# saidwivedi/InteractVLM

Measured on AMD Instinct MI355X. Metric: images/sec end-to-end contact inference, higher is better.
Workload: dtype f16

## Files before the change

### include/ivlm_hip.h

```cpp
#ifndef IVLM_HIP_H
#define IVLM_HIP_H

#include <stddef.h>
#include <stdint.h>

#ifdef __cplusplus
extern "C" {
#endif

#define IVLM_OK 0
#define IVLM_ERR_INVALID_ARG (-1)
#define IVLM_ERR_WORKSPACE (-2)
#define IVLM_ERR_LAUNCH (-3)
#define IVLM_ERR_UNSUPPORTED (-4)

#define IVLM_F32 0
#define IVLM_BF16 1
#define IVLM_BF16_SPLIT 2
#define IVLM_F16 4
#define IVLM_F16_SPLIT 5
#define IVLM_FP8 3

#define IVLM_GEMM_A_F32 1
#define IVLM_GEMM_RES_F32 2
// ... 314 lines not shown
int ivlm_pack_bf12m_fill(const void *w, int N_valid, int n_rows, int K, const int32_t *ebase, const int32_t *patch_ptr, void *Pf, void *Ef,
                         int32_t *patch_col, void *patch_val, ivlm_stream_t stream);
int ivlm_gemv16_bf12m(const float *x, int64_t lda, int M, const void *Pf, const void *Ef, const int32_t *ebase,
                      const int32_t *patch_ptr, const int32_t *patch_col, const void *patch_val, void *C, int64_t ldc, const void *bias,
                      const void *residual, int64_t ldr, int N, int K, int act, int out_f32, const void *rms_w, float rms_eps, int flags,
                      ivlm_stream_t stream);
void ivlm_gemv16_bf12m_tuning(int tiles_per_block);
int ivlm_decode_parts_tuning(int ranges);
void ivlm_gemv1_bf12m_tuning(int wide_max_blocks);
int ivlm_gemv1_bf12m_staging(int form);
int ivlm_unpack_bf12(const void *P, int64_t ldp, const void *E, int64_t lde, const int32_t *ebase, const int32_t *patch_ptr,
                     const int32_t *patch_col, const void *patch_val, int N, int K, void *w_out, ivlm_stream_t stream);

int ivlm_argmax_f32(const float *x, int rows, int cols, int32_t *out, ivlm_stream_t stream);
int ivlm_argmax_f32_bump(const float *x, int rows, int cols, int32_t *out, int32_t *bump, ivlm_stream_t stream);

int ivlm_im2col_nchw(const void *x, void *out, int B, int C, int H, int W, int ks, int stride, int Kpad,
                     ivlm_stream_t stream);
int ivlm_im2col3x3_nhwc(const void *x, void *out, int B, int H, int W, int C, ivlm_stream_t stream);
int ivlm_im2col3x3_nhwc_strided(const void *x, int64_t ldx, void *out, int64_t ldo, int B, int H, int W, int C,
                                ivlm_stream_t stream);
int ivlm_gather_rows(void *dst, int dst_kind, int64_t ldd, const void *src, int src_dtype, int64_t lds, const int32_t *idx,
                     const void *add, int add_dtype, int64_t lda, int64_t rows, int cols, const float *fp8_scale,
                     ivlm_stream_t stream);
int ivlm_amax(const void *x, int dtype, int64_t n, float *out, ivlm_stream_t stream);
int ivlm_add_rows(void *out, int out_kind, const void *a, int a_dtype, const void *b, int b_dtype, int64_t rows, int cols,
                  int64_t b_rows, int op, ivlm_stream_t stream);
int ivlm_fill_rows(void *dst, int64_t ldd, const int32_t *idx, int64_t n_idx, const void *row, int cols,
                   ivlm_stream_t stream);
int ivlm_dense_pe(const void *gauss, void *pe, int pe_dtype, int h, int w, int F, ivlm_stream_t stream);
// ... 181 lines not shown
```

### interactvlm_amd/csrc/elementwise.hip

```cpp
#include "kernels.h"

namespace ivlm {
namespace {

constexpr int kT = 256;

inline int grid_for(int64_t work_items, int max_blocks = 8192) {
    int64_t b = (work_items + kT - 1) / kT;
    if (b < 1) b = 1;
    return (int)(b < max_blocks ? b : max_blocks);
}

__global__ __launch_bounds__(kT) void im2col_nchw_kernel(const bf16_t* __restrict__ x, bf16_t* __restrict__ out, int B,
                                                         int C, int H, int W, int ks, int stride, int Kpad) {
    const int gh = (H - ks) / stride + 1, gw = (W - ks) / stride + 1;
    const int K = C * ks * ks;
    const int64_t total = (int64_t)B * gh * gw * (Kpad >> 3);
    for (int64_t i = (int64_t)blockIdx.x * kT + threadIdx.x; i < total; i += (int64_t)gridDim.x * kT) {
        const int c8 = (int)(i % (Kpad >> 3));
        const int64_t row = i / (Kpad >> 3);
        const int gx = (int)(row % gw), gy = (int)((row / gw) % gh), b = (int)(row / ((int64_t)gw * gh));
        bf16_t v[8];
#pragma unroll
        for (int e = 0; e < 8; ++e) {
// ... 84 lines not shown
    const float inv_scale = scale ? 1.0f / *scale : 1.0f;
    for (int64_t i = (int64_t)blockIdx.x * kT + threadIdx.x; i < total; i += (int64_t)gridDim.x * kT) {
        const int c8 = (int)(i % c8n);
        const int64_t r = i / c8n;
        const int64_t s = idx ? (int64_t)idx[r] : r;
        float v[8] = {0.f, 0.f, 0.f, 0.f, 0.f, 0.f, 0.f, 0.f};
        if (s >= 0) load8(src, src_kind, s * lds_ + c8 * 8, v);
        if (add) {
            float a[8];
            load8(add, add_kind, r * lda + c8 * 8, a);
#pragma unroll
            for (int j = 0; j < 8; ++j) v[j] += a[j];
        }
        store8(dst, dst_kind, r * ldd + c8 * 8, cols, v, inv_scale);
    }
}

__global__ __launch_bounds__(kT) void amax_kernel(const void* __restrict__ x, int kind, int64_t n8, float* __restrict__ out) {
    float m = 0.0f;
    for (int64_t i = (int64_t)blockIdx.x * kT + threadIdx.x; i < n8; i += (int64_t)gridDim.x * kT) {
        float v[8];
        load8(x, kind, i * 8, v);
#pragma unroll
        for (int j = 0; j < 8; ++j) m = fmaxf(m, fabsf(v[j]));
    }
    m = wave_max(m);
    if ((threadIdx.x & 63) == 0) atomicMax(reinterpret_cast<unsigned int*>(out), __float_as_uint(m));
}

__global__ __launch_bounds__(kT) void fill_rows_kernel(bf16_t* __restrict__ dst, int64_t ldd, const int32_t* __restrict__ idx,
// ... 313 lines not shown
    ivlm_enter();
    return ivlm::im2col3x3_nhwc(CBF(x), BF(out), B, H, W, C, ivlm_stream(s));
}
int ivlm_im2col3x3_nhwc_strided(const void* x, int64_t ldx, void* out, int64_t ldo, int B, int H, int W, int C, ivlm_stream_t s) {
    ivlm_enter();
    return ivlm::im2col3x3_nhwc(CBF(x), BF(out), B, H, W, C, ivlm_stream(s), ldx, ldo);
}
int ivlm_gather_rows(void* dst, int dst_kind, int64_t ldd, const void* src, int src_dtype, int64_t lds_, const int32_t* idx,
                     const void* add, int add_dtype, int64_t lda, int64_t rows, int cols, const float* fp8_scale,
                     ivlm_stream_t s) {
    ivlm_enter();
    const int k = dst_kind == IVLM_F32 ? 1 : (dst_kind == IVLM_BF16 ? 0 : (dst_kind == IVLM_BF16_SPLIT ? 2 : (dst_kind == IVLM_FP8 ? 3 : -1)));
    return ivlm::gather_rows(dst, k, ldd, src, src_dtype == IVLM_F32, lds_, idx, add, add_dtype == IVLM_F32, lda, rows, cols,
                             ivlm_stream(s), fp8_scale);
}
int ivlm_amax(const void* x, int dtype, int64_t n, float* out, ivlm_stream_t s) {
    ivlm_enter();
    return ivlm::amax(x, dtype == IVLM_F32, n, out, ivlm_stream(s));
}
int ivlm_add_rows(void* out, int out_kind, const void* a, int a_dtype, const void* b, int b_dtype, int64_t rows, int cols,
                  int64_t b_rows, int op, ivlm_stream_t s) {
    ivlm_enter();
    return ivlm::add_rows(out, out_kind == IVLM_F32 ? 1 : (out_kind == IVLM_BF16 ? 0 : (out_kind == IVLM_BF16_SPLIT ? 2 : -1)),
                          a, a_dtype == IVLM_F32, b, b_dtype == IVLM_F32, rows, cols, b_rows, ivlm_stream(s), op);
}
int ivlm_fill_rows(void* dst, int64_t ldd, const int32_t* idx, int64_t n_idx, const void* row, int cols, ivlm_stream_t s) {
    ivlm_enter();
    return ivlm::fill_rows(BF(dst), ldd, idx, n_idx, CBF(row), cols, ivlm_stream(s));
}
int ivlm_dense_pe(const void* gauss, void* pe, int pe_dtype, int h, int w, int F, ivlm_stream_t s) {
// ... 44 lines not shown
```

### interactvlm_amd/csrc/gemv.hip

```cpp
#include <stdlib.h>

#include <algorithm>

#include "gemv_common.h"

namespace ivlm {
namespace {

constexpr int kMaxM = 8;

__device__ __forceinline__ float dot8(const u32x4_t& w, const u32x4_t& x) {
    float acc = 0.0f;
#pragma unroll
    for (int j = 0; j < 4; ++j) {
        acc += __uint_as_float(w[j] << 16) * __uint_as_float(x[j] << 16);
        acc += __uint_as_float(w[j] & 0xffff0000u) * __uint_as_float(x[j] & 0xffff0000u);
    }
    return acc;
}

__device__ __forceinline__ float dot8f(const u32x4_t& w, const f32x4v_t& xa, const f32x4v_t& xb) {
    float acc = __uint_as_float(w[0] << 16) * xa[0];
    acc = fmaf(__uint_as_float(w[0] & 0xffff0000u), xa[1], acc);
    acc = fmaf(__uint_as_float(w[1] << 16), xa[2], acc);
// ... 295 lines not shown

static int launch_gemv1(const GemmArgs& g, hipStream_t st) {
    int ks = g_gemv1_ksplit > 0 ? g_gemv1_ksplit : 1;
    if (g.act == ACT_SWIGLU || g.K < 2048) ks = 1;
    if (ks == 2) {
        if (g.rms_w) launch_gemv1_ks<true, 2>(g, st);
        else launch_gemv1_ks<false, 2>(g, st);
    } else {
        if (g.rms_w) launch_gemv1_ks<true, 1>(g, st);
        else launch_gemv1_ks<false, 1>(g, st);
    }
    return ivlm_launch_status();
}

__global__ __launch_bounds__(1024) void argmax_kernel(const float* __restrict__ x, int cols, int32_t* __restrict__ out,
                                                      int32_t* __restrict__ bump) {
    __shared__ float sv[16];
    __shared__ int si[16];
    const float* r = x + (int64_t)blockIdx.x * cols;
    float best = -INFINITY;
    int bi = 0x7fffffff;
    auto take = [&](float v, int i) {
        if (v > best || (v == best && i < bi)) {
            best = v;
            bi = i;
        }
    };
    const int head = (int)(((16 - ((uintptr_t)r & 15)) & 15) >> 2);
    const int nhead = head < cols ? head : cols;
    if ((int)threadIdx.x < nhead) take(r[threadIdx.x], threadIdx.x);
    const int nvec = (cols - nhead) >> 2;
    const float4* rv = reinterpret_cast<const float4*>(r + nhead);
    for (int i = threadIdx.x; i < nvec; i += 1024) {
// ... 15 lines not shown
        }
    }
    if ((threadIdx.x & 63) == 0) {
        sv[threadIdx.x >> 6] = best;
        si[threadIdx.x >> 6] = bi;
    }
    __syncthreads();
    if (threadIdx.x == 0) {
        for (int w = 1; w < 16; ++w)
            if (sv[w] > best || (sv[w] == best && si[w] < bi)) {
                best = sv[w];
                bi = si[w];
            }
        out[blockIdx.x] = bi;
        if (bump) bump[blockIdx.x] += 1;
    }
}

}

int g_gemv_max_blocks_per_cu = 0, g_gemv_rows2_min_n = 0;
int g_gemv_legacy = 0;
static int gemv_cu_count() {
    static int cus = 0;
    if (cus == 0) {
        int dev = 0;
        if (hipGetDevice(&dev) != hipSuccess || hipDeviceGetAttribute(&cus, hipDeviceAttributeMultiprocessorCount, dev) != hipSuccess ||
            cus <= 0)
            cus = 256;
    }
// ... 51 lines not shown
        case 7: return launch_gemv<7>(g, st);
        default: return launch_gemv<8>(g, st);
    }
}

int gemv1_fp8w(const GemmArgs& g, hipStream_t st) {
    if (!g.A || !g.W || !g.C || !g.scale_w || g.M != 1 || !g.a_f32 || g.N <= 0 || g.K <= 0) return IVLM_ERR_INVALID_ARG;
    if ((g.K & 15) || (g.ldw & 15) || (size_t)g.K * 4 > 60 * 1024) return IVLM_ERR_UNSUPPORTED;
    if (g.act == ACT_SWIGLU && ((g.N & 1) || g.residual)) return IVLM_ERR_UNSUPPORTED;
    const dim3 grid((g.N + kG1Waves - 1) / kG1Waves), block(64 * kG1Waves);
    if (g.rms_w) ivlm_launch_lds_cap<gemv1_fp8w_kernel<true>>(64 * 1024, grid, block, (size_t)g.K * 4, st, g);
    else ivlm_launch_lds_cap<gemv1_fp8w_kernel<false>>(64 * 1024, grid, block, (size_t)g.K * 4, st, g);
    return ivlm_launch_status();
}

int argmax_f32(const float* x, int rows, int cols, int32_t* out, hipStream_t st, int32_t* bump) {
    if (!x || !out || rows <= 0 || cols <= 0) return IVLM_ERR_INVALID_ARG;
    argmax_kernel<<<rows, 1024, 0, st>>>(x, cols, out, bump);
    return ivlm_launch_status();
}

}

extern "C" int ivlm_gemv_tuning(int max_blocks_per_cu, int rows2_min_n) {
    ivlm::g_gemv_legacy = max_blocks_per_cu < 0 ? 1 : 0;
    ivlm::g_gemv_max_blocks_per_cu = max_blocks_per_cu > 0 ? max_blocks_per_cu : 0;
    ivlm::g_gemv_rows2_min_n = rows2_min_n;
    return 0;
}

extern "C" void ivlm_gemv1_tuning(int ksplit) { ivlm::g_gemv1_ksplit = ksplit; }
extern "C" void ivlm_gemv1_lds_floor(int bytes) { ivlm::g_gemv1_lds_floor = bytes < 0 ? 0 : (bytes > 128 * 1024 ? 128 * 1024 : bytes); }

// ... 5 lines not shown
    g.W = static_cast<const bf16_t*>(Wq);
    g.ldw = ldw;
    g.scale_w = scale_w;
    return ivlm::gemv1_fp8w(g, ivlm_stream(stream));
}

extern "C" int ivlm_argmax_f32(const float* x, int rows, int cols, int32_t* out, ivlm_stream_t stream) {
    ivlm_enter();
    return ivlm::argmax_f32(x, rows, cols, out, ivlm_stream(stream), nullptr);
}

extern "C" int ivlm_argmax_f32_bump(const float* x, int rows, int cols, int32_t* out, int32_t* bump, ivlm_stream_t stream) {
    ivlm_enter();
    return ivlm::argmax_f32(x, rows, cols, out, ivlm_stream(stream), bump);
}
```

### interactvlm_amd/csrc/kernels.h

```cpp
#pragma once
#include "ivlm_common.h"

namespace ivlm {

enum Act : int { ACT_NONE = 0, ACT_GELU = 1, ACT_QUICK_GELU = 2, ACT_RELU = 3, ACT_SILU = 4, ACT_SWIGLU = 5, ACT_SIGMOID = 6 };

struct SplitKFused {
    int32_t* count = nullptr;
    void* C = nullptr;
    const bf16_t* bias = nullptr;
    const bf16_t* residual = nullptr;
    int64_t ldc = 0, ldr = 0, c_lo = 0;
    int res_mod = 0, act = 0, out_f32 = 0, out_f16 = 0, out_split = 0, res_f32 = 0;
};
constexpr int kSplitKCounters = 4096;

struct GemmArgs {
    const bf16_t* A = nullptr;
    const bf16_t* W = nullptr;
    void* C = nullptr;
    const bf16_t* bias = nullptr;
    const bf16_t* residual = nullptr;
    int64_t lda = 0, ldw = 0, ldc = 0, ldr = 0;
    int res_mod = 0;
// ... 20 lines not shown
    float rms_eps = 0.0f;
    SplitKFused sk;
};

GemmArgs gemm_args(const void* A, int64_t lda, const void* W, int64_t ldw, void* C, int64_t ldc, const void* bias, const void* residual,
                   int64_t ldr, int res_mod, int M, int N, int K, int act, int out_f32, int flags, const int32_t* out_rows = nullptr,
                   const int32_t* a_rows = nullptr);
int gemm_bf16(const GemmArgs& g, hipStream_t st);
int gemm_splitk_choice(int M, int N, int K, int act, int has_rms);
int gemm_bf16_splitk(const GemmArgs& g, int splits, float* workspace, size_t ws_bytes, hipStream_t st, int32_t* counters = nullptr);
int linear_bf16(const GemmArgs& g, hipStream_t st);

int layernorm(const void* x, int x_f32, const bf16_t* w, const bf16_t* b, void* y, int y_f32, int64_t rows, int cols, float eps,
              hipStream_t st, int gelu = 0, const int32_t* out_rows = nullptr, const float* fp8_scale = nullptr);
int rmsnorm(const void* x, int x_f32, const bf16_t* w, void* y, int y_f32, int64_t rows, int cols, float eps, hipStream_t st,
            const float* fp8_scale = nullptr);

struct AttnArgs {
    const bf16_t *q, *k, *v;
    bf16_t* o;
    int64_t q_bs, q_hs, q_rs;
    int64_t k_bs, k_hs, k_rs;
    int64_t v_bs, v_hs, v_rs;
    int64_t o_bs, o_hs, o_rs;
    int B, H, Sq, Sk, D;
    float scale;
    int causal;
    int q_pos0;
    const float* rel_h;
    const float* rel_w;
    int rel_kh, rel_kw;
// ... 143 lines not shown
int decode_attn(DecodeAttnForm form, const DecodeAttnArgs& a, hipStream_t st);
bool attn_oproj_fits(int H, int D, int cus);
size_t llama_decode_attn_splitkv_scratch_bytes(int H, int D);
size_t llama_decode_attn_batch_prefix_scratch_bytes(int B, int H, int D);

extern int g_decode_parts_S;
constexpr int kDecodePartsMaxS = 4;
__host__ __device__ constexpr int decode_parts_stride(int D) { return D + 4; }

int spec_accept(const int32_t* amax, const int32_t* fed, const int32_t* nd_dev, int k, int32_t* n_acc, int32_t* tok, int32_t* pos,
                hipStream_t st);

int gemv_bf16(const GemmArgs& g, hipStream_t st);
int gemv1_fp8w(const GemmArgs& g, hipStream_t st);
int gemv_mfma_bf16(const GemmArgs& g, hipStream_t st);
int argmax_f32(const float* x, int rows, int cols, int32_t* out, hipStream_t st, int32_t* bump = nullptr);

}
```

### interactvlm_amd/csrc/norm.hip

```cpp
#include "kernels.h"

namespace ivlm {
namespace {

constexpr int kMaxChunks = 16;

__device__ __forceinline__ void unpack8(const uint4& u, float* f) {
    f[0] = __uint_as_float(u.x << 16); f[1] = __uint_as_float(u.x & 0xffff0000u);
    f[2] = __uint_as_float(u.y << 16); f[3] = __uint_as_float(u.y & 0xffff0000u);
    f[4] = __uint_as_float(u.z << 16); f[5] = __uint_as_float(u.z & 0xffff0000u);
    f[6] = __uint_as_float(u.w << 16); f[7] = __uint_as_float(u.w & 0xffff0000u);
}
__device__ __forceinline__ uint4 pack8(const float* f) {
    return make_uint4(pack_bf16x2(f[0], f[1]), pack_bf16x2(f[2], f[3]), pack_bf16x2(f[4], f[5]),
                      pack_bf16x2(f[6], f[7]));
}

template <bool RMS, int MAXC, bool GELU, bool XF32, bool YF32>
__global__ __launch_bounds__(256) void norm_kernel(const void* __restrict__ xv, const bf16_t* __restrict__ w,
                                                   const bf16_t* __restrict__ b, void* __restrict__ yv, int64_t rows,
                                                   int cols, float eps, const int32_t* __restrict__ out_rows,
                                                   const float* __restrict__ fp8_scale, int y_split) {
    const int lane = threadIdx.x & 63;
    const int64_t row = (int64_t)blockIdx.x * 4 + (threadIdx.x >> 6);
    if (row >= rows) return;
    const int nchunk = cols >> 3;
    const uint4* xr = reinterpret_cast<const uint4*>(static_cast<const bf16_t*>(xv) + row * cols);
    const float4* xr4 = reinterpret_cast<const float4*>(static_cast<const float*>(xv) + row * cols);
    float v[MAXC][8];
    float s = 0.0f;
#pragma unroll
    for (int c = 0; c < MAXC; ++c) {
        const int idx = c * 64 + lane;
        if (idx < nchunk) {
            if (XF32) {
                const float4 a = xr4[2 * idx], bq = xr4[2 * idx + 1];
                v[c][0] = a.x; v[c][1] = a.y; v[c][2] = a.z; v[c][3] = a.w;
                v[c][4] = bq.x; v[c][5] = bq.y; v[c][6] = bq.z; v[c][7] = bq.w;
            } else {
                unpack8(xr[idx], v[c]);
            }
// ... 47 lines not shown
            }
            if (!YF32 && fp8_scale) {
                const float inv = 1.0f / *fp8_scale;
                float cl[8];
#pragma unroll
                for (int j = 0; j < 8; ++j) cl[j] = fminf(fmaxf(o[j] * inv, -448.0f), 448.0f);
                uint32_t a = 0, bq = 0;
                a = __builtin_amdgcn_cvt_pk_fp8_f32(cl[0], cl[1], a, false);
                a = __builtin_amdgcn_cvt_pk_fp8_f32(cl[2], cl[3], a, true);
                bq = __builtin_amdgcn_cvt_pk_fp8_f32(cl[4], cl[5], bq, false);
                bq = __builtin_amdgcn_cvt_pk_fp8_f32(cl[6], cl[7], bq, true);
                reinterpret_cast<uint2*>(static_cast<uint8_t*>(yv) + orow * cols)[idx] = make_uint2(a, bq);
            } else if (YF32) {
                yr4[2 * idx] = make_float4(o[0], o[1], o[2], o[3]);
                yr4[2 * idx + 1] = make_float4(o[4], o[5], o[6], o[7]);
            } else if (y_split == 2) {
                yr[idx] = make_uint4(pack_f16x2(o[0], o[1]), pack_f16x2(o[2], o[3]), pack_f16x2(o[4], o[5]), pack_f16x2(o[6], o[7]));
            } else if (y_split) {
                uint32_t h[4], l[4];
#pragma unroll
                for (int j = 0; j < 4; ++j) split_16x2(o[2 * j], o[2 * j + 1], h[j], l[j], y_split == 3);
                yr[idx] = make_uint4(h[0], h[1], h[2], h[3]);
                yr[nchunk + idx] = make_uint4(l[0], l[1], l[2], l[3]);
            } else {
                yr[idx] = pack8(o);
            }
        }
    }
}

}

template <bool RMS, int MAXC, bool GELU>
static void launch_norm(const void* x, int x_f32, const bf16_t* w, const bf16_t* b, void* y, int y_f32, int64_t rows, int cols,
                        float eps, hipStream_t st, const int32_t* out_rows = nullptr, const float* fp8_scale = nullptr) {
    const unsigned grid = (unsigned)((rows + 3) / 4);
    const int y_split = y_f32 == 2 ? 1 : (y_f32 == 4 ? 2 : (y_f32 == 5 ? 3 : 0));
    if (x_f32 && y_f32 == 1) norm_kernel<RMS, MAXC, GELU, true, true><<<grid, 256, 0, st>>>(x, w, b, y, rows, cols, eps, out_rows, fp8_scale, 0);
    else if (x_f32) norm_kernel<RMS, MAXC, GELU, true, false><<<grid, 256, 0, st>>>(x, w, b, y, rows, cols, eps, out_rows, fp8_scale, y_split);
    else if (y_f32 == 1) norm_kernel<RMS, MAXC, GELU, false, true><<<grid, 256, 0, st>>>(x, w, b, y, rows, cols, eps, out_rows, fp8_scale, 0);
    else norm_kernel<RMS, MAXC, GELU, false, false><<<grid, 256, 0, st>>>(x, w, b, y, rows, cols, eps, out_rows, fp8_scale, y_split);
}

int layernorm(const void* x, int x_f32, const bf16_t* w, const bf16_t* b, void* y, int y_f32, int64_t rows, int cols, float eps,
              hipStream_t st, int gelu, const int32_t* out_rows, const float* fp8_scale) {
    if (!x || !w || !b || !y || rows <= 0 || cols <= 0) return IVLM_ERR_INVALID_ARG;
    if ((cols & 7) || cols > kMaxChunks * 512) return IVLM_ERR_UNSUPPORTED;
    if (gelu) {
        if (cols > 4 * 512) return IVLM_ERR_UNSUPPORTED;
        launch_norm<false, 4, true>(x, x_f32, w, b, y, y_f32, rows, cols, eps, st, out_rows);
    } else if (cols <= 4 * 512) {
        launch_norm<false, 4, false>(x, x_f32, w, b, y, y_f32, rows, cols, eps, st, out_rows, fp8_scale);
    } else {
        launch_norm<false, kMaxChunks, false>(x, x_f32, w, b, y, y_f32, rows, cols, eps, st, out_rows);
    }
    return ivlm_launch_status();
}

int rmsnorm(const void* x, int x_f32, const bf16_t* w, void* y, int y_f32, int64_t rows, int cols, float eps, hipStream_t st,
            const float* fp8_scale) {
    if (!x || !w || !y || rows <= 0 || cols <= 0) return IVLM_ERR_INVALID_ARG;
    if ((cols & 7) || cols > kMaxChunks * 512) return IVLM_ERR_UNSUPPORTED;
    if (fp8_scale && y_f32) return IVLM_ERR_INVALID_ARG;
    if (cols <= 4 * 512) launch_norm<true, 4, false>(x, x_f32, w, nullptr, y, y_f32, rows, cols, eps, st, nullptr, fp8_scale);
    else launch_norm<true, kMaxChunks, false>(x, x_f32, w, nullptr, y, y_f32, rows, cols, eps, st, nullptr, fp8_scale);
    return ivlm_launch_status();
}

}

extern "C" {

int ivlm_layernorm(const void* x, int x_dtype, const void* w, const void* b, void* y, int y_dtype, int64_t rows, int cols,
                   float eps, int gelu, const int32_t* out_rows, const float* fp8_scale, ivlm_stream_t stream) {
    ivlm_enter();
    if ((y_dtype == IVLM_FP8) != (fp8_scale != nullptr)) return IVLM_ERR_INVALID_ARG;
    if (y_dtype == IVLM_FP8 && (gelu || cols > 2048)) return IVLM_ERR_UNSUPPORTED;
    return ivlm::layernorm(x, x_dtype == IVLM_F32, static_cast<const bf16_t*>(w), static_cast<const bf16_t*>(b), y,
                           y_dtype == IVLM_F32 ? 1 : (y_dtype == IVLM_BF16_SPLIT ? 2 : (y_dtype == IVLM_F16 ? 4 : (y_dtype == IVLM_F16_SPLIT ? 5 : 0))),
                           rows, cols, eps, ivlm_stream(stream), gelu, out_rows, fp8_scale);
// ... 2 lines not shown
int ivlm_rmsnorm_fp8(const void* x, int x_dtype, const void* w, void* y, int64_t rows, int cols, float eps, const float* fp8_scale,
                     ivlm_stream_t stream) {
    ivlm_enter();
    if (!fp8_scale) return IVLM_ERR_INVALID_ARG;
    return ivlm::rmsnorm(x, x_dtype == IVLM_F32, static_cast<const bf16_t*>(w), y, 0, rows, cols, eps, ivlm_stream(stream), fp8_scale);
}

int ivlm_rmsnorm(const void* x, int x_dtype, const void* w, void* y, int y_dtype, int64_t rows, int cols, float eps,
                 ivlm_stream_t stream) {
    ivlm_enter();
    return ivlm::rmsnorm(x, x_dtype == IVLM_F32, static_cast<const bf16_t*>(w), y,
                         y_dtype == IVLM_F32 ? 1 : (y_dtype == IVLM_BF16_SPLIT ? 2 : (y_dtype == IVLM_F16 ? 4 : (y_dtype == IVLM_F16_SPLIT ? 5 : 0))),
                         rows, cols, eps, ivlm_stream(stream));
}

}
```

### interactvlm_amd/decoding.py

```python
from __future__ import annotations

import torch

from . import ops
from .constants import IMAGE_TOKEN_INDEX

_ring = None

SHARED_PREFIX_MODES = ("default", "bf16")


def shared_prefix_len(prompts, one_picture, mode="default", fp8=False, image_rows=256, image_id=IMAGE_TOKEN_INDEX):
    prompts = [[int(t) for t in p] for p in prompts]
    B = len(prompts)
    if B < 2 or not one_picture or fp8 or mode not in SHARED_PREFIX_MODES:
        return 0
    n = 0
    while n < min(len(p) for p in prompts) and all(p[n] == prompts[0][n] for p in prompts):
        n += 1
    spliced = lambda ids: len(ids) + sum(image_rows - 1 for t in ids if t == image_id)
    T0 = [spliced(p) for p in prompts]
    P = min(spliced(prompts[0][:n]), min(T0) - 1)
    if P <= 16 or sum(T0) - B * P <= 16:
        return 0
# ... 8 lines not shown


class _Step:
    st = None

    def __init__(self, llm, hidden):
        self.llm, self.hidden = llm, hidden

    def event(self):
        ev = torch.cuda.Event()
        ev.record(torch.cuda.current_stream(self.hidden.device))
        return ev


class SingleGraph(_Step):

    def __init__(self, llm, hidden, T0):
        super().__init__(llm, hidden)
        self.st, self.pos = llm.decode_graph(T0), T0

    def __call__(self, tok, out=None):
        st = self.st
        if isinstance(tok, torch.Tensor):
            st["tok"].copy_(tok)
        else:
            st["tok"].fill_(tok)
        st["graph"].replay()
        self.hidden[self.pos: self.pos + 1].copy_(st["hidden"])
        self.pos += 1
        return st["nxt"].clone() if out is None else out.copy_(st["nxt"])

    def resume(self, n, v):
        self.pos += n
        self.st["pos"].copy_(v["pos"])
        self.st["tok"].copy_(v["tok"])


# ... 54 lines not shown

def greedy(step, nxt, n_seq, eos, forced=None):
    B, n_max = len(n_seq), max(n_seq)
    new = [[] for _ in range(B)]
    done = [False] * B

    def absorb(toks):
        for b in range(B):
            if not done[b]:
                new[b].append(int(toks[b]))
                done[b] = toks[b] == eos or len(new[b]) >= n_seq[b]
        return all(done)

    if forced is not None:
        host, dev = forced
        amax = [nxt]
        for s in range(n_max):
            if absorb([f[s] for f in host]):
                break
            amax.append(step(dev[s]))
        return new, amax
    ring = _id_ring(n_max * B)[: n_max * B].view(n_max, B)
    ids = torch.empty(n_max, B, dtype=torch.int32, device=nxt.device)
    ids[0].copy_(nxt)
    ring[0].copy_(nxt, non_blocking=True)
    evs, amax = [step.event()], []

    def read():
        s = len(amax)
        evs[s].synchronize()
        amax.append(ids[s])
        return absorb(ring[s].tolist())

    for s in range(n_max - 1):
        if s >= 1 and read():
            break
        ring[s + 1].copy_(step(ids[s], out=ids[s + 1]), non_blocking=True)
        evs.append(step.event())
    while not all(done):
        read()
    return new, amax


def speculative(step, nxt, n_max, eos, draft):
    llm = step.llm
    kmax = max(llm.VERIFY_BUCKETS)
    new_ids, amax = [int(nxt.item())], [nxt]
    stats = dict(passes=0, plain_steps=0, proposed=0, accepted=0, pattern=[])
    observe = getattr(draft, "observe", None)
    while new_ids[-1] != eos and len(new_ids) < n_max:
        rem = n_max - len(new_ids)
        prop = [int(t) for t in draft.propose(list(new_ids), kmax)][: min(kmax - 1, rem - 1)]
        m = len(prop)
        if m == 0:
            stats["plain_steps"] += 1
# ... 32 lines not shown
```

### interactvlm_amd/llava.py

```python
from __future__ import annotations

import collections
import os

import torch

from . import _lib, graphs, ops
from .sam import _LN, _Lin, _dev
from .weights import CLIP_PREFIX, ClipCfg, LlamaCfg

BF16 = torch.bfloat16
F32 = torch.float32

_GraphKey = collections.namedtuple("_GraphKey", "batched B precision packed fp8 fused verify prefix", defaults=(False, False))


class ClipTower:

    def __init__(self, w, cfg: ClipCfg, device, prefix=CLIP_PREFIX):
        self.cfg, self.device = cfg, device
        self._graphs = graphs.Cache()
        self._patch_rows = {}
        e = prefix + ".embeddings"
        K = 3 * cfg.patch * cfg.patch
# ... 136 lines not shown
        self.norm = _dev(w[prefix + ".norm.weight"], device)
        self.lm_head = _dev(w["lm_head.weight"], device)
        H, hd = cfg.heads, cfg.hidden // cfg.heads
        self.kcache = torch.zeros(cfg.layers, max_len, H, hd, dtype=BF16, device=device)
        self.vcache = torch.zeros(cfg.layers, max_len, H, hd, dtype=BF16, device=device)
        self.rope = ops.rope_table(max_len, hd, cfg.theta, device)
        self.precision = "default"
        self.decode_splitkv = False
        self.kcache_lo = self.vcache_lo = None
        self._graphs = {}
        self._fused = None
        self.fuse_attn_oproj = bool(os.environ.get("IVLM_FUSE_ATTN_OPROJ"))
        self.decode_packed = os.environ.get("IVLM_DECODE_PACKED", "1") != "0"
        self.decode_attn_parts = os.environ.get("IVLM_DECODE_ATTN_PARTS", "1") != "0"
        self.decode_packed_batch = os.environ.get("IVLM_DECODE_PACKED_BATCH", "1") != "0"

    def prepare(self):
        if self.fp8 or self._calibrating:
            return
        for L in self.layers:
            if self.decode_packed:
                for n in _LayerW.MATS:
                    self._planes(L, n)
            if self.precision == "f16":
                self._f16w(L)
            else:
                for n in _LayerW.MATS:
                    L[n]
        if self.decode_packed and ops.PackedBf12.takes(16, self.cfg.hidden) and getattr(self, "lm_head_p", None) is None:
            self.lm_head_p = ops.PackedBf12(self.lm_head, pad_rows=True)
# ... 223 lines not shown
            t[..., :rows, :, :].copy_(sv)
        self._graphs[key] = st

    def decode_graph(self, pos=None):
        key = self._graph_key(1, batched=False)
        st = self._graphs.get(key)
        if st is None:
            dev, c = self.device, self.cfg
            st = dict(tok=torch.zeros(1, dtype=torch.int32, device=dev), pos=torch.zeros(1, dtype=torch.int32, device=dev),
                      pos64=torch.zeros(1, dtype=torch.int64, device=dev))
            if key.fused:
                st["fused"] = dict(step=torch.zeros(1, dtype=torch.int32, device=dev),
                                   counters=torch.zeros(c.layers, 32, dtype=torch.int32, device=dev),
                                   status=torch.zeros(1, dtype=torch.int32, device=dev),
                                   scratch=torch.zeros(c.layers, c.hidden, dtype=F32, device=dev))
            fz = self._fused = st.get("fused")

            def body():
                e = self.embed_ids(st["tok"])
                h = self._decode_step(e, st["pos"])
                st["hidden"] = h
                st["nxt"] = ops.argmax(self.logits(h), bump=st["pos"])
                if fz is not None:
                    fz["step"].add_(1)

            caches = [self.kcache, self.vcache] + ([self.kcache_lo, self.vcache_lo] if self.precision == "parity" else [])
            counters = [st["pos"], st["pos64"]] + ([fz["step"], fz["counters"]] if fz is not None else [])
            self._capture_decode(key, st, body, caches, counters)
        if pos is not None:
            st["pos"].fill_(pos)
            st["pos64"].fill_(pos)
            if "fused" in st:
                for k in ("step", "counters", "status"):
                    st["fused"][k].zero_()
        return st

    def batch_cache(self, B):
# ... 20 lines not shown
            if getattr(self, "_prefix_scratch", None) is None:
                self._prefix_scratch = ops.decode_attn_prefix_scratch(16, H, hd, self.norm.device)
            return self._decode_layers(x, lin, self._attn_then_o(lin, lambda qkv, li: (
                ops.llama_decode_attn_batch_prefix(qkv, kc[li], vc[li], H, hd, pos_dev, prefix, c.theta, hd ** -0.5, table=self.rope,
                                                   scratch=self._prefix_scratch))))
        return self._decode_layers(x, lin, self._attn_then_o(lin, lambda qkv, li: (
            ops.llama_decode_attn_batch(qkv, kc[li], vc[li], H, hd, pos_dev, c.theta, hd ** -0.5, table=self.rope,
                                        lo=(lo[0][li], lo[1][li]) if lo is not None else None))))

    @staticmethod
    def _planes(L, n):
        if n + "_p" not in L:
            L[n + "_p"] = ops.PackedBf12(L[n]) if ops.PackedBf12.takes(*L[n].shape) else None
        return L[n + "_p"]

    def _decode_layers(self, x, lin, attn_o):
        c = self.cfg
        for li, L in enumerate(self.layers):
            qkv = lin(x, L, "qkv", rms=(L["ln1"], c.eps))
            x = attn_o(qkv, li, L, x)
            h = lin(x, L, "gu", act="swiglu", rms=(L["ln2"], c.eps))
            x = lin(h, L, "down", residual=x)
        return ops.rmsnorm(x, self.norm, c.eps, out_f32=True)

    @staticmethod
    def _attn_then_o(lin, attn):
        return lambda qkv, li, L, x: lin(attn(qkv, li), L, "o", residual=x)

    def _lin(self, planes=None):
        def lin(x, L, n, **kw):
            wp = self._planes(L, n) if planes else None
            if wp is not None and (planes == "any" or wp.frag):
                return ops.linear_bf12(x, wp, **kw)
            return ops.linear(x, L[n], out_f32=True, **kw)
        return lin

    VERIFY_BUCKETS = (4, 8, 16)
# ... 53 lines not shown

            self._capture_decode(key, st, body, [kc, vc] + list(lo or ()), [st["pos"]])
        if pos is not None:
            st["pos"].copy_(pos)
        if prefix is not None:
            st["prefix"].fill_(int(prefix))
        return st

    def _attn_scratch(self):
        if not (self.decode_splitkv or os.environ.get("IVLM_DECODE_SPLITKV", "0") == "1") or self.precision == "parity":
            return None
        if getattr(self, "_dec_scratch", None) is None:
            self._dec_scratch = ops.decode_attn_scratch(self.cfg.heads, self.cfg.hidden // self.cfg.heads, self.norm.device)
        return self._dec_scratch

    def _decode_step(self, x, pos):
        c = self.cfg
        H, hd = c.heads, c.hidden // c.heads
        fz = self._fused if isinstance(pos, torch.Tensor) else None
        if self.fp8:
            lin = lambda x_, L, n, **kw: ops.linear_fp8w(x_, L[n + "_q"], L[n + "_s"], **kw)
            return self._decode_layers(x, lin, self._attn_then_o(lin, lambda qkv, li: ops.llama_decode_attn(
                qkv, self.kcache[li], self.vcache[li], H, hd, pos, c.theta, hd ** -0.5, table=self.rope)))
        kc, vc = self._caches()
        packed = self.decode_packed and fz is None
        lin = self._lin("any" if packed else None)
        attn_o = plain = self._attn_then_o(lin, lambda qkv, li: ops.llama_decode_attn(
            qkv, kc[li], vc[li], H, hd, pos, c.theta, hd ** -0.5, table=self.rope, lo=self._lo(li), scratch=self._attn_scratch()))
        if packed:
            split = self.decode_attn_parts and self._lo(0) is None
            if split and getattr(self, "_parts", None) is None:
                self._parts = torch.zeros(H * 4 * (hd + 4), dtype=F32, device=self.norm.device)

            def attn_o(qkv, li, L, x):
                wo = self._planes(L, "o")
                if not split or wo is None:
                    return plain(qkv, li, L, x)
                ops.llama_decode_attn_parts(qkv, kc[li], vc[li], H, hd, pos, c.theta, hd ** -0.5, self._parts, table=self.rope)
                return ops.linear_bf12(None, wo, residual=x, parts=(self._parts, hd))
        elif fz is not None and self.precision == "default":
            attn_o = lambda qkv, li, L, x: ops.llama_attn_oproj(
                qkv, self.kcache[li], self.vcache[li], L["o"], x, H, hd, pos, fz["step"], fz["counters"][li], fz["status"], c.theta,
                hd ** -0.5, self.rope, fz["scratch"][li])
        return self._decode_layers(x, lin, attn_o)

    def logits(self, hidden_rows):
        if hidden_rows.shape[0] > 16:
            return ops.linear(ops.split_rows(hidden_rows.contiguous()), self.lm_head, out_f32=True, a_split=True)
        if hidden_rows.shape[0] == 1 and self.decode_packed and ops.PackedBf12.takes(16, self.cfg.hidden):
            if getattr(self, "lm_head_p", None) is None:
                self.lm_head_p = ops.PackedBf12(self.lm_head, pad_rows=True)
            return ops.linear_bf12(hidden_rows.contiguous(), self.lm_head_p)
        return ops.linear(hidden_rows, self.lm_head, out_f32=True)
```

### interactvlm_amd/ops.py

```python
from __future__ import annotations

import functools
import os

import torch

from . import _lib
from ._lib import IvlmError, check

IVLM_F32, IVLM_BF16 = 0, 1


def _stream() -> int:
    return torch.cuda.current_stream().cuda_stream


class KernelTimer:

    def __init__(self):
        self.enabled = False
        self.records = {}
        self._hip = None

    def _rt(self):
# ... 787 lines not shown
        call = lambda: check(lib.ivlm_gemm_bf16(q.data_ptr(), q.stride(2), cat.data_ptr(), D, G.data_ptr(), npad, 0, 0, 0, 0,
                                                M, npad, D, 0, 0, H, q.stride(1), 0, M * npad, 0, 0, 0.0, 0, 0, 0, _stream()),
                             "relpos gemm")
        if TIMER.enabled:
            TIMER.time("gemm_bf16_mfma", 2.0 * H * M * npad * D, call, tag=("relpos", M, npad, D))
        else:
            call()
        check(lib.ivlm_relpos_gather(G.data_ptr(), M * npad, npad, B, H, SH, SW, rel_h.data_ptr(), rel_w.data_ptr(), _stream()),
              "relpos_gather")
        return rel_h, rel_w
    check(lib.ivlm_relpos_bias(q.data_ptr(), q.stride(0), q.stride(1), q.stride(2), tab_h.data_ptr(), tab_w.data_ptr(),
                               B, H, SH, SW, D, rel_h.data_ptr(), rel_w.data_ptr(), _stream()), "relpos_bias")
    return rel_h, rel_w


def argmax(logits, bump=None):
    lib = _lib.load()
    logits = _req(logits, torch.float32, "logits")
    rows, cols = logits.shape
    out = torch.empty(rows, dtype=torch.int32, device=logits.device)
    if bump is not None:
        assert bump.dtype == torch.int32 and bump.is_cuda and bump.numel() == rows and bump.is_contiguous()
        check(lib.ivlm_argmax_f32_bump(logits.data_ptr(), rows, cols, out.data_ptr(), bump.data_ptr(), _stream()), "argmax_bump")
        return out
    check(lib.ivlm_argmax_f32(logits.data_ptr(), rows, cols, out.data_ptr(), _stream()), "argmax")
    return out


def im2col_nchw(x, ks, stride, kpad=None):
    lib = _lib.load()
    x = _req(x, BF16, "x")
    B, C, H, W = x.shape
    K = C * ks * ks
    kpad = kpad or ((K + 63) // 64) * 64
    gh, gw = (H - ks) // stride + 1, (W - ks) // stride + 1
    out = torch.empty(B * gh * gw, kpad, dtype=BF16, device=x.device)
    check(lib.ivlm_im2col_nchw(x.data_ptr(), out.data_ptr(), B, C, H, W, ks, stride, kpad, _stream()), "im2col_nchw")
    return out


def im2col3x3_nhwc(x):
# ... 457 lines not shown
```

Before: 10.55.

## Drive decode loop on device so graph replays chain tokens without host copies

```diff
diff --git a/include/ivlm_hip.h b/include/ivlm_hip.h
--- a/include/ivlm_hip.h
+++ b/include/ivlm_hip.h
@@ -352,6 +352,21 @@
 
 int ivlm_argmax_f32(const float *x, int rows, int cols, int32_t *out, ivlm_stream_t stream);
 int ivlm_argmax_f32_bump(const float *x, int rows, int cols, int32_t *out, int32_t *bump, ivlm_stream_t stream);
+
+typedef struct {
+    const int32_t *feed;
+    float *hidden_out;
+    int32_t *ids;
+    int64_t ld_hidden;
+    int32_t n_feed, hidden_rows, n_ids;
+    int32_t step;
+} ivlm_decode_loop;
+size_t ivlm_decode_loop_bytes(void);
+int ivlm_decode_loop_set(void *loop, const int32_t *feed, int n_feed, float *hidden_out, int64_t ld_hidden, int hidden_rows,
+                         int32_t *ids, int n_ids, const int32_t *first, int32_t *tok, int32_t *pos, int pos0, ivlm_stream_t stream);
+int ivlm_rmsnorm_step(const float *x, const void *w, float *y, int cols, float eps, const void *loop, const int32_t *pos,
+                      ivlm_stream_t stream);
+int ivlm_argmax_f32_step(const float *x, int cols, int32_t *out, int32_t *bump, void *loop, int32_t *tok, ivlm_stream_t stream);
 
 int ivlm_im2col_nchw(const void *x, void *out, int B, int C, int H, int W, int ks, int stride, int Kpad,
                      ivlm_stream_t stream);
diff --git a/interactvlm_amd/csrc/elementwise.hip b/interactvlm_amd/csrc/elementwise.hip
--- a/interactvlm_amd/csrc/elementwise.hip
+++ b/interactvlm_amd/csrc/elementwise.hip
@@ -122,6 +122,16 @@
         }
         store8(dst, dst_kind, r * ldd + c8 * 8, cols, v, inv_scale);
     }
+}
+
+__global__ void decode_loop_set_kernel(DecodeLoop* __restrict__ loop, DecodeLoop v, const int32_t* __restrict__ first,
+                                       int32_t* __restrict__ tok, int32_t* __restrict__ pos, int pos0) {
+    if (v.ids) {
+        v.ids[0] = *first;
+        *tok = v.feed ? v.feed[0] : *first;
+    }
+    *loop = v;
+    if (pos) *pos = pos0;
 }
 
 __global__ __launch_bounds__(kT) void amax_kernel(const void* __restrict__ x, int kind, int64_t n8, float* __restrict__ out) {
@@ -465,6 +475,21 @@
     return ivlm::gather_rows(dst, k, ldd, src, src_dtype == IVLM_F32, lds_, idx, add, add_dtype == IVLM_F32, lda, rows, cols,
                              ivlm_stream(s), fp8_scale);
 }
+size_t ivlm_decode_loop_bytes(void) { return sizeof(ivlm_decode_loop); }
+int ivlm_decode_loop_set(void* loop, const int32_t* feed, int n_feed, float* hidden_out, int64_t ld_hidden, int hidden_rows,
+                         int32_t* ids, int n_ids, const int32_t* first, int32_t* tok, int32_t* pos, int pos0, ivlm_stream_t s) {
+    ivlm_enter();
+    if (!loop || ((uintptr_t)loop & 7) || n_feed < 0 || hidden_rows < 0 || n_ids < 0 || pos0 < 0) return IVLM_ERR_INVALID_ARG;
+    if (ids && (n_ids < 1 || (feed && n_feed < 1) || !first || !tok)) return IVLM_ERR_INVALID_ARG;
+    if (ids && hidden_out && (((uintptr_t)hidden_out & 15) || (ld_hidden & 3) || ld_hidden <= 0)) return IVLM_ERR_INVALID_ARG;
+    ivlm_decode_loop v = {};
+    if (ids) {
+        v.feed = feed; v.hidden_out = hidden_out; v.ids = ids; v.ld_hidden = ld_hidden;
+        v.n_feed = feed ? n_feed : 0; v.hidden_rows = hidden_out ? hidden_rows : 0; v.n_ids = n_ids;
+    }
+    ivlm::decode_loop_set_kernel<<<1, 1, 0, ivlm_stream(s)>>>(static_cast<ivlm_decode_loop*>(loop), v, first, tok, pos, pos0);
+    return ivlm_launch_status();
+}
 int ivlm_amax(const void* x, int dtype, int64_t n, float* out, ivlm_stream_t s) {
     ivlm_enter();
     return ivlm::amax(x, dtype == IVLM_F32, n, out, ivlm_stream(s));
diff --git a/interactvlm_amd/csrc/gemv.hip b/interactvlm_amd/csrc/gemv.hip
--- a/interactvlm_amd/csrc/gemv.hip
+++ b/interactvlm_amd/csrc/gemv.hip
@@ -333,9 +333,18 @@
 }
 
 __global__ __launch_bounds__(1024) void argmax_kernel(const float* __restrict__ x, int cols, int32_t* __restrict__ out,
-                                                      int32_t* __restrict__ bump) {
+                                                      int32_t* __restrict__ bump, DecodeLoop* __restrict__ loop,
+                                                      int32_t* __restrict__ tok) {
     __shared__ float sv[16];
     __shared__ int si[16];
+    DecodeLoop d = {};
+    int fed = 0;
+    bool feeds = false;
+    if (loop && threadIdx.x == 0) {
+        d = *loop;
+        feeds = d.ids && d.feed && d.step + 1 >= 0 && d.step + 1 < d.n_feed;
+        if (feeds) fed = d.feed[d.step + 1];
+    }
     const float* r = x + (int64_t)blockIdx.x * cols;
     float best = -INFINITY;
     int bi = 0x7fffffff;
@@ -381,6 +390,12 @@
             }
         out[blockIdx.x] = bi;
         if (bump) bump[blockIdx.x] += 1;
+        if (d.ids) {
+            if (d.step >= 0 && d.step + 1 < d.n_ids) d.ids[d.step + 1] = bi;
+            if (feeds) *tok = fed;
+            else if (!d.feed) *tok = bi;
+            loop->step = d.step + 1;
+        }
     }
 }
 
@@ -462,9 +477,9 @@
     return ivlm_launch_status();
 }
 
-int argmax_f32(const float* x, int rows, int cols, int32_t* out, hipStream_t st, int32_t* bump) {
-    if (!x || !out || rows <= 0 || cols <= 0) return IVLM_ERR_INVALID_ARG;
-    argmax_kernel<<<rows, 1024, 0, st>>>(x, cols, out, bump);
+int argmax_f32(const float* x, int rows, int cols, int32_t* out, hipStream_t st, int32_t* bump, DecodeLoop* loop, int32_t* tok) {
+    if (!x || !out || rows <= 0 || cols <= 0 || (loop && (rows != 1 || !tok))) return IVLM_ERR_INVALID_ARG;
+    argmax_kernel<<<rows, 1024, 0, st>>>(x, cols, out, bump, loop, tok);
     return ivlm_launch_status();
 }
 
@@ -500,3 +515,9 @@
     ivlm_enter();
     return ivlm::argmax_f32(x, rows, cols, out, ivlm_stream(stream), bump);
 }
+
+extern "C" int ivlm_argmax_f32_step(const float* x, int cols, int32_t* out, int32_t* bump, void* loop, int32_t* tok,
+                                    ivlm_stream_t stream) {
+    ivlm_enter();
+    return ivlm::argmax_f32(x, 1, cols, out, ivlm_stream(stream), bump, static_cast<ivlm::DecodeLoop*>(loop), loop ? tok : nullptr);
+}
diff --git a/interactvlm_amd/csrc/kernels.h b/interactvlm_amd/csrc/kernels.h
--- a/interactvlm_amd/csrc/kernels.h
+++ b/interactvlm_amd/csrc/kernels.h
@@ -2,6 +2,8 @@
 #include "ivlm_common.h"
 
 namespace ivlm {
+
+using DecodeLoop = ivlm_decode_loop;
 
 enum Act : int { ACT_NONE = 0, ACT_GELU = 1, ACT_QUICK_GELU = 2, ACT_RELU = 3, ACT_SILU = 4, ACT_SWIGLU = 5, ACT_SIGMOID = 6 };
 
@@ -58,7 +60,7 @@
 int layernorm(const void* x, int x_f32, const bf16_t* w, const bf16_t* b, void* y, int y_f32, int64_t rows, int cols, float eps,
               hipStream_t st, int gelu = 0, const int32_t* out_rows = nullptr, const float* fp8_scale = nullptr);
 int rmsnorm(const void* x, int x_f32, const bf16_t* w, void* y, int y_f32, int64_t rows, int cols, float eps, hipStream_t st,
-            const float* fp8_scale = nullptr);
+            const float* fp8_scale = nullptr, const DecodeLoop* loop = nullptr, const int32_t* loop_pos = nullptr);
 
 struct AttnArgs {
     const bf16_t *q, *k, *v;
@@ -232,6 +234,7 @@
 int gemv_bf16(const GemmArgs& g, hipStream_t st);
 int gemv1_fp8w(const GemmArgs& g, hipStream_t st);
 int gemv_mfma_bf16(const GemmArgs& g, hipStream_t st);
-int argmax_f32(const float* x, int rows, int cols, int32_t* out, hipStream_t st, int32_t* bump = nullptr);
+int argmax_f32(const float* x, int rows, int cols, int32_t* out, hipStream_t st, int32_t* bump = nullptr, DecodeLoop* loop = nullptr,
+               int32_t* tok = nullptr);
 
 }
diff --git a/interactvlm_amd/csrc/norm.hip b/interactvlm_amd/csrc/norm.hip
--- a/interactvlm_amd/csrc/norm.hip
+++ b/interactvlm_amd/csrc/norm.hip
@@ -20,11 +20,17 @@
 __global__ __launch_bounds__(256) void norm_kernel(const void* __restrict__ xv, const bf16_t* __restrict__ w,
                                                    const bf16_t* __restrict__ b, void* __restrict__ yv, int64_t rows,
                                                    int cols, float eps, const int32_t* __restrict__ out_rows,
-                                                   const float* __restrict__ fp8_scale, int y_split) {
+                                                   const float* __restrict__ fp8_scale, int y_split,
+                                                   const DecodeLoop* __restrict__ loop, const int32_t* __restrict__ loop_pos) {
     const int lane = threadIdx.x & 63;
     const int64_t row = (int64_t)blockIdx.x * 4 + (threadIdx.x >> 6);
     if (row >= rows) return;
     const int nchunk = cols >> 3;
+    float4* hr4 = nullptr;
+    if (YF32 && loop && loop->ids && loop->hidden_out) {
+        const int p = *loop_pos;
+        if (p >= 0 && p < loop->hidden_rows) hr4 = reinterpret_cast<float4*>(loop->hidden_out + (int64_t)p * loop->ld_hidden);
+    }
     const uint4* xr = reinterpret_cast<const uint4*>(static_cast<const bf16_t*>(xv) + row * cols);
     const float4* xr4 = reinterpret_cast<const float4*>(static_cast<const float*>(xv) + row * cols);
     float v[MAXC][8];
@@ -102,6 +108,10 @@
             } else if (YF32) {
                 yr4[2 * idx] = make_float4(o[0], o[1], o[2], o[3]);
                 yr4[2 * idx + 1] = make_float4(o[4], o[5], o[6], o[7]);
+                if (hr4) {
+                    hr4[2 * idx] = make_float4(o[0], o[1], o[2], o[3]);
+                    hr4[2 * idx + 1] = make_float4(o[4], o[5], o[6], o[7]);
+                }
             } else if (y_split == 2) {
                 yr[idx] = make_uint4(pack_f16x2(o[0], o[1]), pack_f16x2(o[2], o[3]), pack_f16x2(o[4], o[5]), pack_f16x2(o[6], o[7]));
             } else if (y_split) {
@@ -121,13 +131,14 @@
 
 template <bool RMS, int MAXC, bool GELU>
 static void launch_norm(const void* x, int x_f32, const bf16_t* w, const bf16_t* b, void* y, int y_f32, int64_t rows, int cols,
-                        float eps, hipStream_t st, const int32_t* out_rows = nullptr, const float* fp8_scale = nullptr) {
+                        float eps, hipStream_t st, const int32_t* out_rows = nullptr, const float* fp8_scale = nullptr,
+                        const DecodeLoop* loop = nullptr, const int32_t* loop_pos = nullptr) {
     const unsigned grid = (unsigned)((rows + 3) / 4);
     const int y_split = y_f32 == 2 ? 1 : (y_f32 == 4 ? 2 : (y_f32 == 5 ? 3 : 0));
-    if (x_f32 && y_f32 == 1) norm_kernel<RMS, MAXC, GELU, true, true><<<grid, 256, 0, st>>>(x, w, b, y, rows, cols, eps, out_rows, fp8_scale, 0);
-    else if (x_f32) norm_kernel<RMS, MAXC, GELU, true, false><<<grid, 256, 0, st>>>(x, w, b, y, rows, cols, eps, out_rows, fp8_scale, y_split);
-    else if (y_f32 == 1) norm_kernel<RMS, MAXC, GELU, false, true><<<grid, 256, 0, st>>>(x, w, b, y, rows, cols, eps, out_rows, fp8_scale, 0);
-    else norm_kernel<RMS, MAXC, GELU, false, false><<<grid, 256, 0, st>>>(x, w, b, y, rows, cols, eps, out_rows, fp8_scale, y_split);
+    if (x_f32 && y_f32 == 1) norm_kernel<RMS, MAXC, GELU, true, true><<<grid, 256, 0, st>>>(x, w, b, y, rows, cols, eps, out_rows, fp8_scale, 0, loop, loop_pos);
+    else if (x_f32) norm_kernel<RMS, MAXC, GELU, true, false><<<grid, 256, 0, st>>>(x, w, b, y, rows, cols, eps, out_rows, fp8_scale, y_split, nullptr, nullptr);
+    else if (y_f32 == 1) norm_kernel<RMS, MAXC, GELU, false, true><<<grid, 256, 0, st>>>(x, w, b, y, rows, cols, eps, out_rows, fp8_scale, 0, loop, loop_pos);
+    else norm_kernel<RMS, MAXC, GELU, false, false><<<grid, 256, 0, st>>>(x, w, b, y, rows, cols, eps, out_rows, fp8_scale, y_split, nullptr, nullptr);
 }
 
 int layernorm(const void* x, int x_f32, const bf16_t* w, const bf16_t* b, void* y, int y_f32, int64_t rows, int cols, float eps,
@@ -146,12 +157,13 @@
 }
 
 int rmsnorm(const void* x, int x_f32, const bf16_t* w, void* y, int y_f32, int64_t rows, int cols, float eps, hipStream_t st,
-            const float* fp8_scale) {
+            const float* fp8_scale, const DecodeLoop* loop, const int32_t* loop_pos) {
     if (!x || !w || !y || rows <= 0 || cols <= 0) return IVLM_ERR_INVALID_ARG;
     if ((cols & 7) || cols > kMaxChunks * 512) return IVLM_ERR_UNSUPPORTED;
     if (fp8_scale && y_f32) return IVLM_ERR_INVALID_ARG;
-    if (cols <= 4 * 512) launch_norm<true, 4, false>(x, x_f32, w, nullptr, y, y_f32, rows, cols, eps, st, nullptr, fp8_scale);
-    else launch_norm<true, kMaxChunks, false>(x, x_f32, w, nullptr, y, y_f32, rows, cols, eps, st, nullptr, fp8_scale);
+    if (loop && (!loop_pos || rows != 1 || !x_f32 || y_f32 != 1)) return IVLM_ERR_INVALID_ARG;
+    if (cols <= 4 * 512) launch_norm<true, 4, false>(x, x_f32, w, nullptr, y, y_f32, rows, cols, eps, st, nullptr, fp8_scale, loop, loop_pos);
+    else launch_norm<true, kMaxChunks, false>(x, x_f32, w, nullptr, y, y_f32, rows, cols, eps, st, nullptr, fp8_scale, loop, loop_pos);
     return ivlm_launch_status();
 }
 
@@ -184,4 +196,11 @@
                          rows, cols, eps, ivlm_stream(stream));
 }
 
-}
+int ivlm_rmsnorm_step(const float* x, const void* w, float* y, int cols, float eps, const void* loop, const int32_t* pos,
+                      ivlm_stream_t stream) {
+    ivlm_enter();
+    return ivlm::rmsnorm(x, 1, static_cast<const bf16_t*>(w), y, 1, 1, cols, eps, ivlm_stream(stream), nullptr,
+                         static_cast<const ivlm::DecodeLoop*>(loop), loop ? pos : nullptr);
+}
+
+}
diff --git a/interactvlm_amd/decoding.py b/interactvlm_amd/decoding.py
--- a/interactvlm_amd/decoding.py
+++ b/interactvlm_amd/decoding.py
@@ -46,13 +46,47 @@
 
 
 class SingleGraph(_Step):
+    looping = False
 
     def __init__(self, llm, hidden, T0):
         super().__init__(llm, hidden)
         self.st, self.pos = llm.decode_graph(T0), T0
 
+    def _loop(self):
+        return self.st.get("loop") if getattr(self.llm, "decode_loop", False) else None
+
+    def begin(self, nxt, ids):
+        loop = self._loop()
+        if loop is not None:
+            ops.decode_loop_set(loop, ids=ids.view(-1), first=nxt, tok=self.st["tok"], hidden=self.hidden)
+            self.looping = True
+        return self.looping
+
+    def run(self, nxt, feed, n):
+        loop = self._loop()
+        if n < 1 or loop is None:
+            return None
+        ids = torch.empty(n + 1, dtype=torch.int32, device=nxt.device)
+        ops.decode_loop_set(loop, ids=ids, first=nxt, tok=self.st["tok"], feed=feed.view(-1)[:n], hidden=self.hidden)
+        try:
+            for _ in range(n):
+                self.st["graph"].replay()
+        finally:
+            ops.decode_loop_set(loop)
+        self.pos += n
+        return ids
+
+    def end(self):
+        if self.looping:
+            ops.decode_loop_set(self.st["loop"])
+            self.looping = False
+
     def __call__(self, tok, out=None):
         st = self.st
+        if self.looping:
+            st["graph"].replay()
+            self.pos += 1
+            return out
         if isinstance(tok, torch.Tensor):
             st["tok"].copy_(tok)
         else:
@@ -137,15 +171,19 @@
 
     if forced is not None:
         host, dev = forced
-        amax = [nxt]
-        for s in range(n_max):
-            if absorb([f[s] for f in host]):
-                break
-            amax.append(step(dev[s]))
-        return new, amax
+        n = 0
+        while not absorb([f[n] for f in host]):
+            n += 1
+        run = getattr(step, "run", None)
+        ids = run(nxt, dev, n) if run is not None and B == 1 else None
+        if ids is not None:
+            return new, [ids[s: s + 1] for s in range(n + 1)]
+        return new, [nxt] + [step(dev[s]) for s in range(n)]
     ring = _id_ring(n_max * B)[: n_max * B].view(n_max, B)
     ids = torch.empty(n_max, B, dtype=torch.int32, device=nxt.device)
-    ids[0].copy_(nxt)
+    begin = getattr(step, "begin", None)
+    if begin is None or B != 1 or not begin(nxt, ids):
+        ids[0].copy_(nxt)
     ring[0].copy_(nxt, non_blocking=True)
     evs, amax = [step.event()], []
 
@@ -155,13 +193,17 @@
         amax.append(ids[s])
         return absorb(ring[s].tolist())
 
-    for s in range(n_max - 1):
-        if s >= 1 and read():
-            break
-        ring[s + 1].copy_(step(ids[s], out=ids[s + 1]), non_blocking=True)
-        evs.append(step.event())
-    while not all(done):
-        read()
+    try:
+        for s in range(n_max - 1):
+            if s >= 1 and read():
+                break
+            ring[s + 1].copy_(step(ids[s], out=ids[s + 1]), non_blocking=True)
+            evs.append(step.event())
+        while not all(done):
+            read()
+    finally:
+        if begin is not None:
+            step.end()
     return new, amax
 
 
diff --git a/interactvlm_amd/llava.py b/interactvlm_amd/llava.py
--- a/interactvlm_amd/llava.py
+++ b/interactvlm_amd/llava.py
@@ -174,6 +174,7 @@
         self.decode_packed = os.environ.get("IVLM_DECODE_PACKED", "1") != "0"
         self.decode_attn_parts = os.environ.get("IVLM_DECODE_ATTN_PARTS", "1") != "0"
         self.decode_packed_batch = os.environ.get("IVLM_DECODE_PACKED_BATCH", "1") != "0"
+        self.decode_loop = os.environ.get("IVLM_DECODE_LOOP", "1") != "0"
 
     def prepare(self):
         if self.fp8 or self._calibrating:
@@ -427,13 +428,18 @@
                                    counters=torch.zeros(c.layers, 32, dtype=torch.int32, device=dev),
                                    status=torch.zeros(1, dtype=torch.int32, device=dev),
                                    scratch=torch.zeros(c.layers, c.hidden, dtype=F32, device=dev))
+            else:
+                st["loop"] = ops.decode_loop(dev)
             fz = self._fused = st.get("fused")
+            loop = st.get("loop")
 
             def body():
-                e = self.embed_ids(st["tok"])
-                h = self._decode_step(e, st["pos"])
+                h = self._decode_step(self.embed_ids(st["tok"]), st["pos"], loop)
                 st["hidden"] = h
-                st["nxt"] = ops.argmax(self.logits(h), bump=st["pos"])
+                if loop is None:
+                    st["nxt"] = ops.argmax(self.logits(h), bump=st["pos"])
+                else:
+                    st["nxt"] = ops.argmax(self.logits(h), bump=st["pos"], loop=(loop, st["tok"]))
                 if fz is not None:
                     fz["step"].add_(1)
 
@@ -484,13 +490,15 @@
             L[n + "_p"] = ops.PackedBf12(L[n]) if ops.PackedBf12.takes(*L[n].shape) else None
         return L[n + "_p"]
 
-    def _decode_layers(self, x, lin, attn_o):
+    def _decode_layers(self, x, lin, attn_o, loop=None):
         c = self.cfg
         for li, L in enumerate(self.layers):
             qkv = lin(x, L, "qkv", rms=(L["ln1"], c.eps))
             x = attn_o(qkv, li, L, x)
             h = lin(x, L, "gu", act="swiglu", rms=(L["ln2"], c.eps))
             x = lin(h, L, "down", residual=x)
+        if loop is not None:
+            return ops.rmsnorm_step(x, self.norm, c.eps, *loop)
         return ops.rmsnorm(x, self.norm, c.eps, out_f32=True)
 
     @staticmethod
@@ -574,14 +582,15 @@
             self._dec_scratch = ops.decode_attn_scratch(self.cfg.heads, self.cfg.hidden // self.cfg.heads, self.norm.device)
         return self._dec_scratch
 
-    def _decode_step(self, x, pos):
+    def _decode_step(self, x, pos, loop=None):
         c = self.cfg
         H, hd = c.heads, c.hidden // c.heads
         fz = self._fused if isinstance(pos, torch.Tensor) else None
+        loop = None if loop is None else (loop, pos)
         if self.fp8:
             lin = lambda x_, L, n, **kw: ops.linear_fp8w(x_, L[n + "_q"], L[n + "_s"], **kw)
             return self._decode_layers(x, lin, self._attn_then_o(lin, lambda qkv, li: ops.llama_decode_attn(
-                qkv, self.kcache[li], self.vcache[li], H, hd, pos, c.theta, hd ** -0.5, table=self.rope)))
+                qkv, self.kcache[li], self.vcache[li], H, hd, pos, c.theta, hd ** -0.5, table=self.rope)), loop)
         kc, vc = self._caches()
         packed = self.decode_packed and fz is None
         lin = self._lin("any" if packed else None)
@@ -602,7 +611,7 @@
             attn_o = lambda qkv, li, L, x: ops.llama_attn_oproj(
                 qkv, self.kcache[li], self.vcache[li], L["o"], x, H, hd, pos, fz["step"], fz["counters"][li], fz["status"], c.theta,
                 hd ** -0.5, self.rope, fz["scratch"][li])
-        return self._decode_layers(x, lin, attn_o)
+        return self._decode_layers(x, lin, attn_o, loop)
 
     def logits(self, hidden_rows):
         if hidden_rows.shape[0] > 16:
diff --git a/interactvlm_amd/ops.py b/interactvlm_amd/ops.py
--- a/interactvlm_amd/ops.py
+++ b/interactvlm_amd/ops.py
@@ -825,17 +825,48 @@
     return rel_h, rel_w
 
 
-def argmax(logits, bump=None):
+def argmax(logits, bump=None, loop=None):
     lib = _lib.load()
     logits = _req(logits, torch.float32, "logits")
     rows, cols = logits.shape
     out = torch.empty(rows, dtype=torch.int32, device=logits.device)
+    if loop is not None:
+        assert rows == 1 and (bump is None or (bump.dtype == torch.int32 and bump.is_cuda and bump.numel() == 1))
+        check(lib.ivlm_argmax_f32_step(logits.data_ptr(), cols, out.data_ptr(), _p(bump), loop[0].data_ptr(), loop[1].data_ptr(),
+                                       _stream()), "argmax_step")
+        return out
     if bump is not None:
         assert bump.dtype == torch.int32 and bump.is_cuda and bump.numel() == rows and bump.is_contiguous()
         check(lib.ivlm_argmax_f32_bump(logits.data_ptr(), rows, cols, out.data_ptr(), bump.data_ptr(), _stream()), "argmax_bump")
         return out
     check(lib.ivlm_argmax_f32(logits.data_ptr(), rows, cols, out.data_ptr(), _stream()), "argmax")
     return out
+
+
+def decode_loop(device):
+    return torch.zeros(_lib.load().ivlm_decode_loop_bytes(), dtype=U8, device=device)
+
+
+def decode_loop_set(loop, ids=None, first=None, tok=None, feed=None, hidden=None, pos=None, pos0=0):
+    lib = _lib.load()
+    assert ids is None or (first is not None and tok is not None)
+    for t in (ids, first, tok, feed, pos):
+        assert t is None or (t.dtype == torch.int32 and t.is_cuda and t.is_contiguous())
+    assert hidden is None or (hidden.dtype == F32 and hidden.is_cuda and hidden.dim() == 2 and hidden.stride(1) == 1)
+    check(lib.ivlm_decode_loop_set(loop.data_ptr(), _p(feed), 0 if feed is None else feed.numel(), _p(hidden),
+                                   0 if hidden is None else hidden.stride(0), 0 if hidden is None else hidden.shape[0], _p(ids),
+                                   0 if ids is None else ids.numel(), _p(first), _p(tok), _p(pos), int(pos0), _stream()),
+          "decode_loop_set")
+
+
+def rmsnorm_step(x, weight, eps, loop=None, pos=None):
+    lib = _lib.load()
+    x = _req(x, F32, "x")
+    assert x.numel() == x.shape[-1] and (loop is None or (pos is not None and pos.dtype == torch.int32 and pos.is_cuda))
+    y = torch.empty(x.shape, dtype=F32, device=x.device)
+    check(lib.ivlm_rmsnorm_step(x.data_ptr(), weight.data_ptr(), y.data_ptr(), x.shape[-1], float(eps), _p(loop), _p(pos), _stream()),
+          "rmsnorm_step")
+    return y
 
 
 def im2col_nchw(x, ks, stride, kpad=None):
```

Measured after the change: 10.56 (median of 3 runs). No clear change (+0.0%).
